# mpizenberg/visual-odometry-rs

Hardware: AMD Instinct MI355X
Metric: frame-pairs/sec (640x480, 6 pyramid levels) (higher is better)
Workload: dtype f32

## Files before the change

include/vors_hip.h:

```cpp
#ifndef VORS_HIP_H
#define VORS_HIP_H

#include <stddef.h>
#include <stdint.h>

#ifdef __cplusplus
extern "C" {
#endif

typedef enum vors_status {
    VORS_OK = 0,
    VORS_ERR_INVALID_ARGUMENT = -1,
    VORS_ERR_NO_DEVICE = -2,
    VORS_ERR_HIP = -3,
    VORS_ERR_PYRAMID_TOO_SHORT = -4,
    VORS_ERR_UNSUPPORTED = -5
} vors_status;

enum { VORS_ROW_MAJOR = 0, VORS_COL_MAJOR = 1 };

enum { VORS_CANDIDATES_COARSE_TO_FINE = 0, VORS_CANDIDATES_DENSE = 1, VORS_CANDIDATES_DSO = 2 };

enum { VORS_ARITH_REFERENCE = 0, VORS_ARITH_EXACT = 1, VORS_ARITH_FUSED = 2 };

// ... 181 lines not shown
                                 int32_t* d_out_status, vors_pair_stats* d_out_stats , void* hip_stream, int64_t* ticket);
vors_status vors_pipeline_wait(vors_pipeline* p, int64_t ticket, void* hip_stream, int host_sync);
vors_status vors_pipeline_drain(vors_pipeline* p, void* hip_stream, int host_sync);
void vors_pipeline_destroy(vors_pipeline* p);

vors_status vors_batch_get_keyframe_image(vors_batch* b, int pair, int level, uint8_t* out, int* rows, int* cols);
vors_status vors_batch_get_current_image(vors_batch* b, int pair, int level, uint8_t* out, int* rows, int* cols);
vors_status vors_batch_get_points(vors_batch* b, int pair, int level, int capacity, int32_t* xy, float* idepth, float* jac,
                                  uint8_t* tmpl, int* n);

typedef struct vors_multi vors_multi;
vors_status vors_multi_create(const vors_config* cfg, int n_devices, const int* device_ids, int max_pairs_per_device, int rows, int cols,
                              vors_multi** out);
int vors_multi_device_count(const vors_multi* m);
int vors_multi_rccl_version(const vors_multi* m);
vors_status vors_multi_shard(const vors_multi* m, int n_pairs_total, int k, int* first, int* count);
vors_status vors_multi_track_pairs(vors_multi* m, int n_pairs_total, const uint8_t* const* d_kf_gray, const uint16_t* const* d_kf_depth,
                                   const uint8_t* const* d_cur_gray, float* out_poses7, int32_t* out_status);
vors_status vors_multi_track_pairs_host(vors_multi* m, int n_pairs_total, const uint8_t* kf_gray, const uint16_t* kf_depth,
                                        const uint8_t* cur_gray, float* out_poses7, int32_t* out_status);
void vors_multi_destroy(vors_multi* m);

vors_status vors_batch_eval_level(vors_batch* b, int pair, int level, const float model7[7], int arithmetic, float sums29[29]);

enum { VORS_EVAL_FULL = 0, VORS_EVAL_ENERGY = 1 };

vors_status vors_batch_eval_pairs(vors_batch* b, int n_pairs, int level, int models_per_pair, const void* d_models, size_t model_stride_bytes,
                                  int arithmetic, int what, float* d_sums29, void* hip_stream);

vors_status vors_batch_pose_information(vors_batch* b, int n_pairs, int level, const void* d_models, size_t model_stride_bytes,
                                        float* d_info36, float* d_cov36, float* d_sigma2, int32_t* d_flags, void* hip_stream);

vors_status vors_pose_information_from_sums(const float sums29[29], float info36[36], float cov36[36], float* sigma2, int32_t* flag);

#define VORS_RESIDUAL_BINS 256
vors_status vors_batch_residual_maps(vors_batch* b, int n_pairs, int level, const void* d_models, size_t model_stride_bytes,
                                     float* d_residuals, float* d_warp_uv, uint32_t* d_hist, float* d_scale, void* hip_stream);

vors_status vors_residual_scale_from_hist(const uint32_t hist[VORS_RESIDUAL_BINS], float* median_abs, float* sigma_mad, uint32_t* n_inside);

vors_status vors_batch_reproject_depth(vors_batch* b, int n_pairs, int level, const void* d_models, size_t model_stride_bytes,
                                       const uint16_t* d_cur_depth , float tol_m,
                                       float* d_pred_z, uint16_t* d_pred_depth, float* d_depth_residual, uint32_t* d_counts,
                                       void* hip_stream);

vors_status vors_batch_point_cloud(vors_batch* b, int n_pairs, int level,
// ... 176 lines not shown
```

visual-odometry-rs_amd/csrc/batch.cpp:

```cpp
#include <algorithm>
#include <cstdlib>
#include <cstring>
#include <memory>

#include "host_common.h"

using namespace vors;

#ifndef VORS_FUSED_EXACT_POINTS_DEFAULT
#define VORS_FUSED_EXACT_POINTS_DEFAULT 2500
#endif
static vors_status build_geom(const vors_config* cfg, int rows, int cols, Geom* g) {
    if (!cfg) return fail(VORS_ERR_INVALID_ARGUMENT, "cfg is NULL");
    if (cfg->nb_levels < 1 || cfg->nb_levels > VORS_MAX_LEVELS)
        return fail(VORS_ERR_INVALID_ARGUMENT, "nb_levels must be in [1, " + std::to_string(VORS_MAX_LEVELS) + "]");
    if (rows < 2 || cols < 2 || rows > 65535 || cols > 65535) return fail(VORS_ERR_INVALID_ARGUMENT, "rows/cols must be in [2, 65535]");
    if ((long long)rows * cols > (1ll << 28))
        return fail(VORS_ERR_INVALID_ARGUMENT, "rows * cols must not exceed 2^28 pixels");
    if (cfg->candidates_mode != VORS_CANDIDATES_COARSE_TO_FINE && cfg->candidates_mode != VORS_CANDIDATES_DENSE &&
        cfg->candidates_mode != VORS_CANDIDATES_DSO)
        return fail(VORS_ERR_INVALID_ARGUMENT, "unknown candidates_mode");
    if (cfg->candidates_diff_threshold < 0 || cfg->candidates_diff_threshold > 65535)
        return fail(VORS_ERR_INVALID_ARGUMENT, "candidates_diff_threshold must fit u16");
    std::memset(g, 0, sizeof(*g));
// ... 93 lines not shown
    p.ws.mask_stride = g.S0 + g.S0 / 4 + g.S0 / 16 + 64;
    p.ws.list_cap = (g.S0 / 16 + g.S0 / 64 + g.S0 / 256 + 1024 + 3) & ~3;
    int off = 0;
    for (int l = 0; l < g.L; ++l) {
        p.pp.off[l] = off;
        if (l >= 1) off += (g.lv[l].rows * g.lv[l].cols + 3) & ~3;
    }
    p.pp.stride = off > 0 ? off : 4;
    int coff = 0;
    for (int l = 0; l < g.L; ++l) {
        p.pp.chunk_off[l] = coff;
        coff += (g.lv[l].rows * g.lv[l].cols + VORS_CHUNK_PX - 1) / VORS_CHUNK_PX;
    }
    p.pp.chunk_off[g.L] = p.pp.chunks_total = coff;
    return p;
}

struct SplitPlan {
    bool present;
    int slots;
    int chunks;
    int n_split, rounds;
    bool side_lane;
};
static SplitPlan plan_split(const Geom& g, int max_pairs) {
    SplitPlan p{};
    p.present = g.mode == VORS_CANDIDATES_DENSE && !(getenv("VORS_LM_SPLIT") && atoi(getenv("VORS_LM_SPLIT")) == 0);
    if (!p.present) return p;
    int chunks = max_pairs >= 1024 ? 64 : (max_pairs >= 512 ? 128 : 256);
    chunks = std::max(4, std::min(chunks, g.S0 / 2400));
    if (const char* ev = getenv("VORS_LM_CHUNKS")) chunks = std::max(4, atoi(ev));
    p.slots = chunks;
    int n_split = 0;
    for (int l = 0; l < g.L; ++l)
        if ((long long)g.lv[l].rows * g.lv[l].cols >= 65536) n_split = l + 1;
    p.n_split = getenv("VORS_LM_SPLIT_LEVELS") ? atoi(getenv("VORS_LM_SPLIT_LEVELS")) : std::max(1, n_split);
    p.n_split = std::max(1, std::min(p.n_split, g.L));
    if (g.arith == VORS_ARITH_FUSED)
        while (p.n_split > 0 && g.lv[p.n_split - 1].rows * g.lv[p.n_split - 1].cols <= g.fused_exact_points) p.n_split -= 1;
    const int ns = p.n_split;
    p.rounds = getenv("VORS_LM_SPLIT_ROUNDS") ? atoi(getenv("VORS_LM_SPLIT_ROUNDS")) : (max_pairs >= 512 ? (ns <= 1 ? 12 : 26) : 4 * ns + 8);
    p.chunks = p.n_split == 0 ? 0 : chunks;
    const int side_from = (getenv("VORS_LM_SIDE") && atoi(getenv("VORS_LM_SIDE")) == 1) ? 512 : 2048;
    p.side_lane = p.chunks > 0 && p.n_split == 2 && max_pairs >= side_from && !(getenv("VORS_LM_SIDE") && atoi(getenv("VORS_LM_SIDE")) == 0);
    if (p.side_lane && !getenv("VORS_LM_SPLIT_ROUNDS")) p.rounds = 10;
    return p;
}

static void allocate_workspaces(vors_batch* b) {
    const Geom& g = b->g;
    DeviceResources& own = b->own;
    const size_t np = (size_t)b->max_pairs;
    const size_t slots = np * (size_t)g.slots_total;
    own.alloc(&b->kf_upper, np * g.upper_stride);
    own.alloc(&b->cur_upper, np * g.upper_stride);
    if (g.mode == VORS_CANDIDATES_DENSE) {
        own.alloc(&b->rec.IZ, slots);
        own.alloc(&b->rec.V, slots);
        own.alloc(&b->rec.n_used, np * VORS_MAX_LEVELS);
        if (plan_ref_dense_planes(g)) {
            RefDensePlanes& t = b->rec.dense_t;
            own.alloc(&t.recs, np * ((size_t)g.S0 + g.upper_stride));
            own.alloc(&t.n_valid, np * VORS_MAX_LEVELS);
            own.alloc(&t.cur0, np * g.S0);
            own.alloc(&t.curu, np * g.upper_stride);
        }
    } else {
        own.alloc(&b->rec.S, slots);
// ... 17 lines not shown
        b->dso = plan.ws;
        b->pp = plan.pp;
        own.alloc(&b->dso.gmag, np * g.S0);
        own.alloc(&b->dso.median, np * b->dso.n_regions);
        own.alloc(&b->dso.thresh, np * b->dso.n_regions);
        own.alloc(&b->dso.max_g, np * b->dso.max_stride);
        own.alloc(&b->dso.max_pos, np * b->dso.max_stride);
        own.alloc(&b->dso.mask1, np * b->dso.mask_stride);
        own.alloc(&b->dso.picked, np * g.S0);
        own.alloc(&b->dso.state, np);
        if (own.err == hipSuccess) own.err = hipMemset(b->dso.state, 0, np * sizeof(DsoState));
        own.alloc(&b->dso.pick_list, np * (size_t)b->dso.list_cap);
        own.alloc(&b->mask0, np * g.S0);
        own.alloc(&b->pp.iz, np * b->pp.stride);
        own.alloc(&b->pp.v, np * b->pp.stride);
        own.alloc(&b->pp.counts, np * b->pp.chunks_total);
    }
    const SplitPlan sp = plan_split(g, b->max_pairs);
    if (sp.present) {
        LmSplitWs& ws = b->split;
        ws.chunks = sp.chunks;
        ws.n_split = sp.n_split;
        ws.rounds = sp.rounds;
        ws.cap = b->max_pairs;
        own.alloc(&ws.state, np);
        own.alloc(&ws.partials, np * sp.slots * 32);
        own.alloc(&ws.list[0], np);
        own.alloc(&ws.list[1], np);
        own.alloc(&ws.count, (size_t)SPLIT_COUNT_INTS);
        ws.side_round = sp.side_lane ? 1 : -1;
        if (sp.side_lane) {
            own.alloc(&ws.side_list, np);
            own.alloc(&ws.join_list, np);
            own.stream(&ws.side_stream, hipStreamNonBlocking);
            own.event(&ws.ev_fork, hipEventDisableTiming);
            own.event(&ws.ev_join, hipEventDisableTiming);
        }
    }
    if (g.mode == VORS_CANDIDATES_DENSE) {
        float2* lut = nullptr;
        own.alloc(&lut, (size_t)65536);
        b->rec.LUT = lut;
    }
}

vors_status check_stream(const vors_batch* b, hipStream_t s) {
// ... 307 lines not shown
    return VORS_OK;
}

vors_status vors_batch_eval_level(vors_batch* b, int pair, int level, const float model7[7], int arithmetic, float sums29[29]) {
    if (!b || !model7 || !sums29) return fail(VORS_ERR_INVALID_ARGUMENT, "NULL argument");
    vors_status st = check_eval(b, pair, level, arithmetic);
    if (st != VORS_OK) return st;
    DeviceGuard guard(b->device);
    DevBuf d_model, d_out;
    HIP_TRY(d_model.alloc(7 * sizeof(float)));
    HIP_TRY(d_out.alloc(32 * sizeof(float)));
    HIP_TRY(hipDeviceSynchronize());
    HIP_TRY(hipMemcpy(d_model.p, model7, 7 * sizeof(float), hipMemcpyHostToDevice));
    const EvalCall call{batch_scene(b, true), pair, level, d_model.as<float>(), d_out.as<float>()};
    if (arithmetic == VORS_ARITH_REFERENCE)
        launch_lm_eval_level_reference(b->g, call, nullptr);
    else if (arithmetic == VORS_ARITH_FUSED) launch_lm_eval_level_fused(b->g, call, nullptr);
    else launch_lm_eval_level_exact(b->g, call, nullptr);
    HIP_TRY(hipDeviceSynchronize());
    HIP_TRY(hipMemcpy(sums29, d_out.p, 29 * sizeof(float), hipMemcpyDeviceToHost));
    return VORS_OK;
}

static vors_status ensure_eval_pairs_ws(vors_batch* b) {
    EvalPairsWs& ws = b->eval_pairs;
    if (ws.items > 0) return VORS_OK;
    const int items = std::min(std::max(b->max_pairs, 256), 32768);
    int chunks = 1;
    for (int l = 0; l < b->g.L; ++l) chunks = std::max(chunks, eval_pairs_chunks(b->g, l));
    if (!ws.partials) b->own.alloc(&ws.partials, (size_t)items * chunks * 32);
    if (!ws.fctx) b->own.alloc(&ws.fctx, (size_t)items);
    if (!ws.sums29) b->own.alloc(&ws.sums29, (size_t)b->max_pairs * 29);
    if (b->own.err != hipSuccess) return own_alloc_failed(b, "evaluation workspace");
    ws.items = items;
    ws.chunks = chunks;
    return VORS_OK;
}

static vors_status batch_eval_pairs(vors_batch* b, int n_pairs, int level, int models_per_pair, const void* d_models, size_t model_stride_bytes,
                                    int arithmetic, int what, float* d_sums29, hipStream_t s) {
    vors_status st = ensure_eval_pairs_ws(b);
    if (st != VORS_OK) return st;
    EvalPairsCall call{batch_scene(b, true)};
    call.n_items = n_pairs * models_per_pair;
    call.models_per_pair = models_per_pair;
    call.lvl = level;
// ... 252 lines not shown
```

visual-odometry-rs_amd/csrc/engine.h:

```cpp
#pragma once
#include <hip/hip_runtime.h>
#include <stdint.h>

#include <type_traits>

#include "../../include/vors_hip.h"
#include "lie.h"

namespace vors {

struct LevelGeom {
    int rows, cols;
    int img_off;
    int n_slots;
    int slot_off;
    Intr k;
    FastDiv fu, fv;
    double inv_fu_d, inv_fv_d;
    float inv_fu, inv_fv, s_fuv;
};

struct Geom {
    int L;
    int mode;
// ... 71 lines not shown
};
struct DsoWs {
    uint8_t* gmag;
    uint16_t* median;
    uint16_t* thresh;
    uint8_t* max_g;
    uint32_t* max_pos;
    uint8_t* mask1;
    uint8_t* picked;
    DsoState* state;
    uint32_t* pick_list;
    int n_regions, max_stride, mask_stride, list_cap;
};
struct LmSplitState {
    float entry[7];
    float model[7];
    float cand[7];
    float sums[32];
    float cur_energy, lm_coef;
    int nb_iter;
    int n_full;
    int lvl;
    int phase;
    int went_well;
    float fctx[21];
    int fctx_exact;
};
#define VORS_SPLIT_MAX_ROUNDS 62
struct LmSplitWs {
    LmSplitState* state;
    float* partials;
    int* list[2];
    int* count;
    int cap;
    int chunks;
    int chunks0;
    int n_split;
    int rounds;
    int side_round;
    int* side_list;
    int* join_list;
    hipStream_t side_stream;
    hipEvent_t ev_fork, ev_join;
};
#define SPLIT_SIDE_COUNT (2 * (VORS_SPLIT_MAX_ROUNDS + 2))
#define SPLIT_JOIN_COUNT (2 * (VORS_SPLIT_MAX_ROUNDS + 2) + 1)
#define SPLIT_COUNT_INTS (2 * (VORS_SPLIT_MAX_ROUNDS + 2) + 2)

struct PixelPlanes {
    float* iz;
    float* v;
    int off[VORS_MAX_LEVELS];
    int stride;
    int* counts;
    int chunk_off[VORS_MAX_LEVELS + 1];
    int chunks_total;
};
constexpr int VORS_CHUNK_PX = 4096;

struct Pyramid {
    const uint8_t* level0;
// ... 472 lines not shown
```

visual-odometry-rs_amd/csrc/lm_kernels.hip:

```cpp
#include <hip/hip_runtime.h>

#include <algorithm>
#include <type_traits>

#include "lm_sources.h"

#ifndef VORS_FUSED
#define VORS_FUSED 0
#endif

namespace vors {

constexpr bool kFused = VORS_FUSED != 0;

#ifndef VORS_ABL_EXACT_STEP
#define VORS_ABL_EXACT_STEP 0
#endif
#ifndef VORS_ABL_IEEE_IDEPTH
#define VORS_ABL_IEEE_IDEPTH 0
#endif
#ifndef VORS_ABL_WIDE_IDENTITY
#define VORS_ABL_WIDE_IDENTITY 0
#endif
#ifndef VORS_ABL_IEEE_RCP
// ... 676 lines not shown
#pragma unroll
    for (int k = 0; k < 8; ++k) c[k] += __int_as_float(__builtin_amdgcn_mov_dpp(__float_as_int(c[k]), 0x104, 0xf, 0xf, true));
#pragma unroll
    for (int k = 0; k < 8; ++k) c[k] += __int_as_float(__builtin_amdgcn_mov_dpp(__float_as_int(c[k]), 0x108, 0xf, 0xf, true));
    if ((threadIdx.x & 15) < 4) {
        float4* p = reinterpret_cast<float4*>(s.part + (threadIdx.x >> 4) * 32 + (threadIdx.x & 3) * 8);
        p[0] = make_float4(c[0], c[1], c[2], c[3]);
        p[1] = make_float4(c[4], c[5], c[6], c[7]);
    }
    __syncthreads();
    if (threadIdx.x < NACC) {
        const int slot = (threadIdx.x & 3) * 8 + (threadIdx.x >> 2);
        float t = 0.f;
#pragma unroll 8
        for (int w = 0; w < BLOCK / 16; ++w) t += s.part[w * 32 + slot];
        s.sums[dst][threadIdx.x] = t;
    }
    __syncthreads();
}

template <int BLOCK>
__device__ __forceinline__ void block_sum2(float& a, float& b, LmShared& s);

__device__ __forceinline__ bool lm_step_fast(const float* h, const float* g, const Iso& model, float lm_coef, Iso* out) {
    float a[6][6], inv[6];
#pragma unroll
    for (int r = 0; r < 6; ++r)
#pragma unroll
        for (int c = 0; c <= r; ++c) a[r][c] = h[r * 6 + c];
    const float scale = 1.0f + lm_coef;
#pragma unroll
    for (int r = 0; r < 6; ++r) a[r][r] *= scale;
    bool ok = true;
#pragma unroll
    for (int j = 0; j < 6; ++j) {
#pragma unroll
        for (int k = 0; k < j; ++k) {
#pragma unroll
            for (int i = j; i < 6; ++i) a[i][j] = fmaf(-a[j][k], a[i][k], a[i][j]);
        }
        const float diag = a[j][j];
        ok = ok && (diag > 0.0f);
        inv[j] = __builtin_amdgcn_rsqf(diag);
        a[j][j] = diag * inv[j];
#pragma unroll
        for (int i = j + 1; i < 6; ++i) a[i][j] *= inv[j];
    }
    if (!ok) return false;
    float b[6];
#pragma unroll
    for (int i = 0; i < 6; ++i) b[i] = g[i];
#pragma unroll
    for (int i = 0; i < 6; ++i) {
        b[i] *= inv[i];
#pragma unroll
        for (int k = i + 1; k < 6; ++k) b[k] = fmaf(-b[i], a[k][i], b[k]);
    }
#pragma unroll
    for (int i = 5; i >= 0; --i) {
        float acc = b[i];
#pragma unroll
        for (int k = i + 1; k < 6; ++k) acc = fmaf(-a[k][i], b[k], acc);
        b[i] = acc * inv[i];
    }
    const float vx = b[0], vy = b[1], vz = b[2], wx = b[3], wy = b[4], wz = b[5];
    const float theta_2 = fmaf(wz, wz, fmaf(wy, wy, wx * wx));
    float real_factor, imag_factor, c1, c2;
    if (theta_2 < 1e-2f * 1e-2f) {
        real_factor = fmaf(-0.125f, theta_2, 1.0f);
        imag_factor = fmaf(-(1.0f / 48.0f), theta_2, 0.5f);
        c1 = fmaf(-(1.0f / 24.0f), theta_2, 0.5f);
        c2 = fmaf(-(1.0f / 120.0f), theta_2, 1.0f / 6.0f);
    } else {
        const float theta = sqrtf(theta_2), half_theta = 0.5f * theta, rt2 = 1.0f / theta_2;
        real_factor = cosf(half_theta);
        imag_factor = sinf(half_theta) / theta;
        const float sh = sinf(half_theta);
        c1 = 2.0f * sh * sh * rt2;
        c2 = (theta - sinf(theta)) * rt2 / theta;
    }
    const float w11 = wx * wx, w12 = wx * wy, w13 = wx * wz, w22 = wy * wy, w23 = wy * wz, w33 = wz * wz;
    Iso dw;
    dw.t.x = fmaf(fmaf(c2, -w22 - w33, 1.0f), vx, fmaf(fmaf(c2, w12, -c1 * wz), vy, fmaf(c2, w13, c1 * wy) * vz));
    dw.t.y = fmaf(fmaf(c2, w12, c1 * wz), vx, fmaf(fmaf(c2, -w11 - w33, 1.0f), vy, fmaf(c2, w23, -c1 * wx) * vz));
    dw.t.z = fmaf(fmaf(c2, w13, -c1 * wy), vx, fmaf(fmaf(c2, w23, c1 * wx), vy, fmaf(c2, -w11 - w22, 1.0f) * vz));
    const Quat q{imag_factor * wx, imag_factor * wy, imag_factor * wz, real_factor};
// ... 449 lines not shown
#define VORS_SPLIT_ENERGY_WAVES 8
#endif
#ifndef VORS_FSPLIT_WAVES
#define VORS_FSPLIT_WAVES 5
#endif
#ifndef VORS_FSPLIT_ENERGY_WAVES
#define VORS_FSPLIT_ENERGY_WAVES 8
#endif
template <bool HUBER, bool ENERGY, bool FUSED>
__global__ __launch_bounds__(SPLIT_BLOCK) __attribute__((amdgpu_waves_per_eu(FUSED ? (ENERGY ? VORS_FSPLIT_ENERGY_WAVES : VORS_FSPLIT_WAVES) : (ENERGY ? VORS_SPLIT_ENERGY_WAVES : VORS_SPLIT_WAVES)))) void
lm_split_eval_kernel(Geom g, const uint8_t* __restrict__ cur0, const uint8_t* __restrict__ curu, const uint8_t* __restrict__ kf0,
                     const uint8_t* __restrict__ kfu, const uint16_t* __restrict__ kf_depth, Records rec, LmSplitWs ws, int round) {
    __shared__ LmShared s;
    const int n_active = ws.count[(ENERGY ? SPLIT_COUNT_STRIDE : 0) + round], n_items = n_active * ws.chunks0;
    const int* list = ws.list[round & 1];
    for (int item = blockIdx.x; item < n_items; item += gridDim.x) {
        const int chunk = item / n_active, a = item - chunk * n_active;
        const int pair = __builtin_amdgcn_readfirstlane(ENERGY ? list[ws.cap - 1 - a] : list[a]);
        const LmSplitState* st = ws.state + pair;
        const int lvl = __builtin_amdgcn_readfirstlane(st->lvl);
        const int chunks = split_chunks(ws, lvl);
        if (chunk >= chunks) continue;
        const int phase = __builtin_amdgcn_readfirstlane(st->phase);
        const Iso model = iso_uniform(iso_load(phase == 1 ? st->cand : st->model));
        const ImgCtx c = level_ctx(g, cur0, curu, pair, lvl);
        float acc[NACC];
        float* out = ws.partials + ((size_t)pair * ws.chunks + chunk) * 32;
        with_level_source<true, true, FUSED>(g, lvl, pair, kf0, kfu, kf_depth, rec, [&](const auto& src, int n_units) {
            const LevelCut cut = level_cut(n_units, chunk, chunks);
            eval_accumulate<SPLIT_BLOCK, HUBER, false, typename std::remove_cv<typename std::remove_reference<decltype(src)>::type>::type, ENERGY>(
                src, cut.last, c, model, acc, nullptr, cut.first, FUSED ? st : nullptr);
        });
        if (ENERGY) {
            float e = acc[0], cnt = acc[1];
            block_sum2<SPLIT_BLOCK>(e, cnt, s);
            if (threadIdx.x == 0) {
                out[0] = e;
                out[1] = cnt;
            }
        } else {
            block_reduce<SPLIT_BLOCK>(acc, s, 0);
            if (threadIdx.x < NACC) out[threadIdx.x] = s.sums[0][threadIdx.x];
        }
        __syncthreads();
    }
}
#if !VORS_FUSED
template <int STEP_WAVES>
__global__ __launch_bounds__(64 * STEP_WAVES) void lm_split_step_kernel(Geom g, LmSplitWs ws, vors_pair_stats* __restrict__ out_stats, int round, int late,
                                                                        int next_late) {
    __shared__ float red_all[STEP_WAVES][32];
    __shared__ int s_kind[STEP_WAVES], s_base[3];
    const int n_active = split_n_active(ws, round);
    const int wave = threadIdx.x >> 6, lane = threadIdx.x & 63;
    float* red = red_all[wave];
    for (int a0 = blockIdx.x * STEP_WAVES; a0 < n_active; a0 += gridDim.x * STEP_WAVES) {
        const int a = a0 + wave;
        const bool live = a < n_active;
        int append_kind = -1;
        const int pair = split_active(ws, round, live ? a : 0);
        LmSplitState* st = ws.state + pair;
        const int lvl = st->lvl;
        const int chunks = split_chunks(ws, lvl);
        const int phase = st->phase;
        const bool have_full = phase != 1 || late;
        const int n_sums = have_full ? NACC : 2;
        if (live && lane < n_sums) {
            const float* pp = ws.partials + (size_t)pair * ws.chunks * 32 + lane;
            float t = 0.f;
            int ch = 0;
            for (; ch + 8 <= chunks; ch += 8) {
                float v[8];
#pragma unroll
                for (int q = 0; q < 8; ++q) v[q] = pp[(ch + q) * 32];
#pragma unroll
                for (int q = 0; q < 8; ++q) t += v[q];
            }
            for (; ch < chunks; ++ch) t += pp[ch * 32];
            red[lane] = t;
        }
        __syncthreads();
        if (live && lane == 0) {
            const float energy = red[0] / red[1];
            Iso cur_model = iso_load(st->model);
            float lm_coef = st->lm_coef, cur_energy = st->cur_energy;
            int nb_iter = st->nb_iter;
            int n_full = st->n_full;
            bool take = false, done = false, need_gh = false;
            if (phase == 0) {
                take = true;
                cur_energy = energy;
                lm_coef = 0.1f;
                nb_iter = 0;
                n_full = 1;
            } else if (phase == 4) {
                take = true;
            } else {
                const LmVerdict v = lm_verdict(energy, cur_energy, nb_iter, lm_coef);
                if (lm_accepted(v)) {
                    n_full += 1;
                    cur_energy = energy;
                    cur_model = iso_load(st->cand);
                }
                if (lm_stops(v)) done = true;
                else if (lm_accepted(v) && have_full) take = true;
                else if (lm_accepted(v)) need_gh = true;
            }
            bool again = false;
            if (done) {
                if (out_stats) store_level_stats(out_stats, pair, lvl, true, nb_iter, n_full, cur_energy);
                iso_store(cur_model, st->model);
                if (lvl > 0) {
                    iso_store(cur_model, st->entry);
                    st->lvl = lvl - 1;
                    st->phase = 0;
                    nb_iter = 0;
                    n_full = 0;
                    again = true;
                } else {
                    st->phase = 2;
                }
            } else if (need_gh) {
                iso_store(cur_model, st->model);
                st->cur_energy = cur_energy;
                st->lm_coef = lm_coef;
                st->phase = 4;
                again = true;
            } else {
                if (take) {
                    for (int q = 0; q < NACC; ++q) st->sums[q] = red[q];
                    iso_store(cur_model, st->model);
                    st->cur_energy = cur_energy;
                }
                st->lm_coef = lm_coef;
                nb_iter += 1;
                const float* sm = take ? red : st->sums;
                float h[36], gr[6];
                for (int q = 0; q < 6; ++q) gr[q] = sm[2 + q];
                int k = 8;
                for (int q = 0; q < 6; ++q)
                    for (int r = q; r < 6; ++r) {
                        h[q * 6 + r] = sm[k];
                        h[r * 6 + q] = sm[k];
                        ++k;
                    }
                Iso cand;
                if ((g.arith == VORS_ARITH_FUSED && !VORS_ABL_EXACT_STEP) ? lm_step_fast(h, gr, cur_model, lm_coef, &cand) : lm_step(h, gr, cur_model, lm_coef, &cand)) {
                    iso_store(cand, st->cand);
                    st->phase = 1;
                    again = true;
                } else {
                    for (int q = 0; q < 7; ++q) st->model[q] = st->entry[q];
                    st->went_well = 0;
                    st->phase = 2;
                    if (out_stats) zero_level_stats_below(out_stats, pair, lvl + 1);
                }
            }
            st->nb_iter = nb_iter;
            st->n_full = n_full;
            if (again && g.arith == VORS_ARITH_FUSED) store_fused_ctx(g, st->lvl, iso_load(st->phase == 1 ? st->cand : st->model), st);
            if (again) append_kind = (round == ws.side_round && st->lvl > 0) ? 2 : ((st->phase == 1 && !next_late) ? 1 : 0);
        }
        if (lane == 0) s_kind[wave] = append_kind;
        __syncthreads();
        if (threadIdx.x == 0) {
            int n_full = 0, n_energy = 0, n_side = 0;
            for (int w = 0; w < STEP_WAVES; ++w) {
                n_full += s_kind[w] == 0 ? 1 : 0;
                n_energy += s_kind[w] == 1 ? 1 : 0;
                n_side += s_kind[w] == 2 ? 1 : 0;
            }
            s_base[0] = n_full ? atomicAdd(&ws.count[round + 1], n_full) : 0;
            s_base[1] = n_energy ? atomicAdd(&ws.count[SPLIT_COUNT_STRIDE + round + 1], n_energy) : 0;
            s_base[2] = n_side ? atomicAdd(&ws.count[SPLIT_SIDE_COUNT], n_side) : 0;
        }
        __syncthreads();
        if (lane == 0 && append_kind >= 0) {
            int rank = 0;
            for (int w = 0; w < wave; ++w) rank += s_kind[w] == append_kind ? 1 : 0;
            if (append_kind == 2) ws.side_list[s_base[2] + rank] = pair;
            else if (append_kind == 1) ws.list[(round + 1) & 1][ws.cap - 1 - (s_base[1] + rank)] = pair;
            else ws.list[(round + 1) & 1][s_base[0] + rank] = pair;
        }
        __syncthreads();
    }
}

__global__ __launch_bounds__(256) void lm_split_merge_kernel(LmSplitWs ws, int round) {
    const int n = ws.count[SPLIT_JOIN_COUNT];
    for (int i = threadIdx.x; i < n; i += 256) ws.list[round & 1][atomicAdd(&ws.count[round], 1)] = ws.join_list[i];
}
void launch_lm_split_merge(LmSplitWs ws, int round, hipStream_t s) { hipLaunchKernelGGL(lm_split_merge_kernel, dim3(1), dim3(256), 0, s, ws, round); }
void launch_lm_split_step(const Geom& g, LmSplitWs ws, vors_pair_stats* out_stats, int round, int late, int next_late, int grid, hipStream_t s) {
    if (grid >= 1024 && !late)
        hipLaunchKernelGGL(lm_split_step_kernel<8>, dim3((grid + 7) / 8), dim3(512), 0, s, g, ws, out_stats, round, late, next_late);
    else
        hipLaunchKernelGGL(lm_split_step_kernel<1>, dim3(grid), dim3(64), 0, s, g, ws, out_stats, round, late, next_late);
}
#else
void launch_lm_split_merge(LmSplitWs ws, int round, hipStream_t s);
void launch_lm_split_step(const Geom& g, LmSplitWs ws, vors_pair_stats* out_stats, int round, int late, int next_late, int grid, hipStream_t s);
#endif

static void launch_lm_track_mode(const Geom& g, const TrackCall& call, int n_groups, int block, LmTrackMode mode, const LmSplitWs& split, hipStream_t s) {
    with_bool(g.mode == VORS_CANDIDATES_DENSE, [&](auto dense) {
        with_bool(g.huber_delta > 0.f, [&](auto huber) {
            with_largest_reached<1024, 512, 256, 128, 64>(block, [&](auto b) {
                constexpr int BLOCK = decltype(b)::value;
                launch_track(lm_track_kernel<BLOCK, decltype(huber)::value, decltype(dense)::value, kFused>, dim3(n_groups), dim3(BLOCK), 0, s, g, call,
                             (int)mode, split);
            });
        });
    });
}

template <bool HUBER, bool DENSE, bool FUSED>
__global__ __launch_bounds__(256) void lm_eval_level_kernel(Geom g, const uint8_t* __restrict__ cur0, const uint8_t* __restrict__ curu,
                                                             const uint8_t* __restrict__ kf0, const uint8_t* __restrict__ kfu,
                                                             const uint16_t* __restrict__ kf_depth, Records rec, int pair, int lvl,
                                                             const float* __restrict__ model7, float* __restrict__ out29) {
    __shared__ LmShared s;
    const Iso model = iso_uniform(iso_load(model7));
    const ImgCtx c = level_ctx(g, cur0, curu, pair, lvl);
    float acc[NACC];
// ... 101 lines not shown
                                      dim3(chunks, n), dim3(EVALP_BLOCK), s, g, call, item0);
                });
            });
        });
        if (chunks > 1) launch_lm_eval_pairs_sum(a, n, chunks, s);
    }
}

#if VORS_FUSED
#define VORS_LAUNCH_LM_TRACK launch_lm_track_fused
#else
#define VORS_LAUNCH_LM_TRACK launch_lm_track_exact
#endif
void VORS_LAUNCH_LM_TRACK(const Geom& g_in, const TrackCall& call, int block, LmSplitWs split, hipStream_t s) {
    const Geom g = launch_geom(g_in, call);
    const int n_pairs = call.n_pairs;
    if (g.mode != VORS_CANDIDATES_DENSE || split.chunks <= 0) {
        launch_lm_track_mode(g, call, n_pairs, block, LM_WHOLE_TRACK, split, s);
        return;
    }
    split.n_split = std::max(1, std::min(split.n_split, g.L));
    split.rounds = std::max(1, std::min(split.rounds, VORS_SPLIT_MAX_ROUNDS));
    (void)hipMemsetAsync(split.count, 0, SPLIT_COUNT_INTS * sizeof(int), s);
    const int join_round = split.side_round >= 0 ? std::min(split.side_round + 3, split.rounds) : -1;
    launch_lm_track_mode(g, call, n_pairs, block, LM_COARSE_LEVELS, split, s);
    const int base_chunks = std::max(1, split.chunks / 4);
    for (int r = 0; r < split.rounds; ++r) {
        static const int late_env = getenv("VORS_LM_LATE_FROM") ? atoi(getenv("VORS_LM_LATE_FROM")) : -1;
        const int late_from = late_env >= 0 ? late_env : 2 * split.n_split + 2;
        const int late = r >= late_from, next_late = r + 1 >= late_from;
        if (r == join_round) {
            (void)hipStreamWaitEvent(s, split.ev_join, 0);
            launch_lm_split_merge(split, r, s);
        }
        static const int late_chunks_env = getenv("VORS_LM_LATE_CHUNKS") ? atoi(getenv("VORS_LM_LATE_CHUNKS")) : 0;
        split.chunks0 = late ? (late_chunks_env > 0 ? std::min(late_chunks_env, split.chunks) : split.chunks) : base_chunks;
        const int full = n_pairs * split.chunks0;
        const int shrink = r < 2 * split.n_split ? 1 : (late ? 16 : 2);
        const int grid = std::max(std::min(full, 256), full / shrink);
        const int minor = std::max(std::min(full, 256), grid / 8);
        const int grid_full = late ? grid : ((r & 1) ? minor : grid), grid_energy = (r & 1) ? grid : minor;
        with_bool(g.huber_delta > 0.f, [&](auto huber) {
            constexpr bool HUBER = decltype(huber)::value;
            launch_on_scene(lm_split_eval_kernel<HUBER, false, kFused>, dim3(grid_full), dim3(SPLIT_BLOCK), 0, s, g, call, split, r);
            if (!late && r > 0) launch_on_scene(lm_split_eval_kernel<HUBER, true, kFused>, dim3(grid_energy), dim3(SPLIT_BLOCK), 0, s, g, call, split, r);
        });
        launch_lm_split_step(g, split, call.out_stats, r, late, next_late, std::max(1, n_pairs / shrink), s);
        if (r == split.side_round) {
            (void)hipEventRecord(split.ev_fork, s);
            (void)hipStreamWaitEvent(split.side_stream, split.ev_fork, 0);
            launch_lm_track_mode(g, call, n_pairs, 1024, LM_SIDE_LANE, split, split.side_stream);
            (void)hipEventRecord(split.ev_join, split.side_stream);
        }
    }
    if (join_round == split.rounds) {
        (void)hipStreamWaitEvent(s, split.ev_join, 0);
        launch_lm_split_merge(split, split.rounds, s);
    }
    launch_lm_track_mode(g, call, n_pairs, 1024, LM_STRAGGLERS, split, s);
    launch_lm_track_mode(g, call, n_pairs, block, LM_EPILOGUE, split, s);
}

#if !VORS_FUSED
void launch_lm_track(const Geom& g, const TrackCall& call, int block, LmSplitWs split, hipStream_t s) {
    if (g.arith == VORS_ARITH_FUSED) launch_lm_track_fused(g, call, block, split, s);
    else launch_lm_track_exact(g, call, block, split, s);
}

#define OP_BLOCK 256
__global__ void records_from_obs_kernel(Intr k, int rows, int cols, const uint8_t* __restrict__ tmpl, int n,
// ... 96 lines not shown
```

visual-odometry-rs_amd/vors_amd/__init__.py:

```python
import ctypes as C
import os
import sys

import numpy as np

_HERE = os.path.dirname(os.path.abspath(__file__))
LIB_PATH = os.environ.get("VORS_HIP_LIB") or os.path.join(_HERE, "libvors_hip.so")
MAX_LEVELS = 8
RESIDUAL_BINS = 256
RENDER_COUNTS = 4
NORMAL_COUNTS = 3
ICP_ITERATIONS, ICP_CONVERGED, ICP_TOO_FEW, ICP_SINGULAR = 0, 1, 2, 3

ROW_MAJOR, COL_MAJOR = 0, 1
CANDIDATES_COARSE_TO_FINE, CANDIDATES_DENSE, CANDIDATES_DSO = 0, 1, 2
TRACK_OK, TRACK_OPTIMIZER_FAILED_POSE_KEPT = 0, 1
ARITH_REFERENCE, ARITH_EXACT, ARITH_FUSED = 0, 1, 2


class VorsError(RuntimeError):
    pass


class vors_config(C.Structure):
# ... 41 lines not shown
    _fields_ = [
        ("cu", C.c_float), ("cv", C.c_float), ("fu", C.c_float), ("fv", C.c_float), ("skew", C.c_float),
        ("rows", C.c_int32), ("cols", C.c_int32),
        ("template_", C.POINTER(C.c_uint8)),
        ("image", C.POINTER(C.c_uint8)),
        ("n", C.c_int32),
        ("coordinates", C.POINTER(C.c_int32)),
        ("_z_candidates", C.POINTER(C.c_float)),
        ("jacobians", C.POINTER(C.c_float)),
        ("huber_delta", C.c_float),
        ("arithmetic", C.c_int32),
    ]


EXPORTED_SYMBOLS = [
    "vors_last_error", "vors_device_count", "vors_device_info", "vors_abi_version", "vors_selfcheck_isqrt",
    "vors_tracker_create", "vors_tracker_track", "vors_tracker_track_checked", "vors_tracker_current_frame", "vors_tracker_last_stats",
    "vors_tracker_keyframe", "vors_tracker_enable_depth_filter", "vors_tracker_enable_map", "vors_tracker_read_map", "vors_tracker_enable_map_voxels",
    "vors_tracker_read_map_voxels", "vors_tracker_render_map", "vors_tracker_destroy",
    "vors_track_pairs",
    "vors_batch_create", "vors_batch_create_on", "vors_batch_device", "vors_batch_track_pairs", "vors_batch_prepare_keyframes", "vors_batch_track_current",
    "vors_batch_workspace_bytes", "vors_batch_enable_kernel_timing", "vors_batch_kernel_times", "vors_batch_last_kernel_ms",
    "vors_batch_destroy",
    "vors_batch_get_keyframe_image", "vors_batch_get_current_image", "vors_batch_get_points", "vors_batch_eval_level",
    "vors_batch_eval_pairs", "vors_batch_pose_information", "vors_pose_information_from_sums",
    "vors_batch_residual_maps", "vors_residual_scale_from_hist",
    "vors_batch_reproject_depth", "vors_to_depth", "vors_from_depth",
    "vors_batch_point_cloud", "vors_camera_back_project", "vors_camera_project",
    "vors_batch_fuse_depth", "vors_fuse_depth_pixels",
    "vors_render_points", "vors_render_points_host", "vors_trackers_render_map",
    "vors_depth_normals", "vors_points_normals", "vors_depth_normals_host", "vors_trackers_enable_map_normals", "vors_trackers_map_normals",
    "vors_icp_workspace_bytes", "vors_icp_points", "vors_icp_points_host", "vors_trackers_icp_map",
    "vors_icp_points_robust", "vors_icp_points_robust_host", "vors_trackers_icp_map_robust",
    "vors_icp_points_joint", "vors_icp_points_joint_host", "vors_trackers_icp_map_joint",
    "vors_tracker_enable_map_normals", "vors_tracker_read_map_normals",
    "vors_trackers_enable_map_icp", "vors_trackers_map_icp", "vors_tracker_enable_map_icp", "vors_tracker_read_map_icp",
    "vors_map_icp_window_host", "vors_map_icp_verdict_host",
    "vors_icp_condition_from_sums", "vors_icp_condition", "vors_trackers_enable_map_icp_joint", "vors_trackers_map_icp_joint",
    "vors_tracker_enable_map_icp_joint", "vors_tracker_read_map_icp_joint", "vors_map_icp_verdict_joint_host",
    "vors_trackers_enable_map_icp_means", "vors_trackers_map_icp_means", "vors_tracker_enable_map_icp_means", "vors_tracker_read_map_icp_means",
    "vors_lm_eval", "vors_lm_step", "vors_lm_solve",
    "vors_ref_sincos", "vors_se3_exp", "vors_se3_log", "vors_so3_exp", "vors_so3_log", "vors_iso_mul", "vors_iso_inverse",
    "vors_synth_render_pairs",
    "vors_multi_create", "vors_multi_device_count", "vors_multi_shard", "vors_multi_track_pairs", "vors_multi_track_pairs_host",
    "vors_multi_destroy", "vors_multi_rccl_version",
    "vors_trackers_create", "vors_trackers_create_on", "vors_trackers_count", "vors_trackers_init", "vors_trackers_track", "vors_trackers_state",
    "vors_trackers_current_frames", "vors_trackers_last_stats", "vors_trackers_enable_kernel_timing", "vors_trackers_kernel_times", "vors_trackers_destroy",
# ... 119 lines not shown
        _lib.vors_tracker_read_map_icp_means.argtypes = [vp, vp]
        _lib.vors_voxel_keys.argtypes = [f, vp, i, vp]
        _lib.vors_voxel_keys.restype = None
        _lib.vors_synth_render_frames.argtypes = [i, vp, vp, vp, i, i, vp, i, vp, vp, vp]
        _lib.vors_batch_track_pairs.argtypes = [vp, i, vp, vp, vp, vp, vp, vp, vp, vp]
        _lib.vors_pipeline_create.argtypes = [i, C.POINTER(vors_config), i, i, i, i, C.POINTER(vp)]
        _lib.vors_pipeline_submit.argtypes = [vp, i, vp, vp, vp, vp, vp, vp, vp, vp, C.POINTER(C.c_int64)]
        _lib.vors_pipeline_wait.argtypes = [vp, C.c_int64, vp, i]
        _lib.vors_pipeline_drain.argtypes = [vp, vp, i]
        _lib.vors_pipeline_destroy.argtypes = [vp]
        _lib.vors_pipeline_destroy.restype = None
        _lib.vors_batch_prepare_keyframes.argtypes = [vp, i, vp, vp, vp]
        _lib.vors_batch_track_current.argtypes = [vp, i, vp, vp, vp, vp, vp, vp]
        _lib.vors_batch_workspace_bytes.argtypes = [vp, C.POINTER(C.c_uint64)]
        _lib.vors_batch_enable_kernel_timing.argtypes = [vp, i]
        _lib.vors_batch_kernel_times.argtypes = [vp, i, vp, i, C.POINTER(i)]
        _lib.vors_batch_last_kernel_ms.argtypes = [vp, C.POINTER(f), C.POINTER(f), C.POINTER(f)]
        _lib.vors_batch_destroy.argtypes = [vp]
        _lib.vors_batch_destroy.restype = None
        _lib.vors_batch_get_keyframe_image.argtypes = [vp, i, i, vp, C.POINTER(i), C.POINTER(i)]
        _lib.vors_batch_get_current_image.argtypes = [vp, i, i, vp, C.POINTER(i), C.POINTER(i)]
        _lib.vors_batch_get_points.argtypes = [vp, i, i, i, vp, vp, vp, vp, C.POINTER(i)]
        _lib.vors_batch_eval_level.argtypes = [vp, i, i, vp, i, vp]
        _lib.vors_batch_eval_pairs.argtypes = [vp, i, i, i, vp, C.c_size_t, i, i, vp, vp]
        _lib.vors_batch_pose_information.argtypes = [vp, i, i, vp, C.c_size_t, vp, vp, vp, vp, vp]
        _lib.vors_pose_information_from_sums.argtypes = [vp, vp, vp, C.POINTER(f), C.POINTER(C.c_int32)]
        _lib.vors_batch_residual_maps.argtypes = [vp, i, i, vp, C.c_size_t, vp, vp, vp, vp, vp]
        _lib.vors_residual_scale_from_hist.argtypes = [vp, C.POINTER(f), C.POINTER(f), C.POINTER(C.c_uint32)]
        _lib.vors_batch_reproject_depth.argtypes = [vp, i, i, vp, C.c_size_t, vp, f, vp, vp, vp, vp, vp]
        for name in ("vors_to_depth", "vors_from_depth"):
            getattr(_lib, name).argtypes = [f, vp, i, vp]
            getattr(_lib, name).restype = None
        _lib.vors_batch_point_cloud.argtypes = [vp, i, i, vp, C.c_size_t, vp, i, vp, vp, vp, vp, vp]
        _lib.vors_camera_back_project.argtypes = [vp, vp, vp, vp, i, vp]
        _lib.vors_camera_back_project.restype = None
        _lib.vors_camera_project.argtypes = [vp, vp, vp, i, vp]
        _lib.vors_camera_project.restype = None
        _lib.vors_batch_fuse_depth.argtypes = [vp, i, vp, C.c_size_t, vp, f, vp, i, i, vp, vp, vp, vp, vp]
        _lib.vors_fuse_depth_pixels.argtypes = [f, f, i, i, C.c_size_t, vp, vp, vp, C.c_size_t, vp, vp, vp]
        _lib.vors_lm_eval.argtypes = [C.POINTER(vors_obs), vp, C.POINTER(f), C.POINTER(C.c_int32), vp, vp, vp]
        _lib.vors_ref_sincos.argtypes = [vp, i, vp, vp]
        _lib.vors_ref_sincos.restype = None
        _lib.vors_lm_step.argtypes = [vp, vp, vp, f, vp, C.POINTER(i)]
        _lib.vors_lm_solve.argtypes = [C.POINTER(vors_obs), vp, vp, C.POINTER(C.c_int32), C.POINTER(f), C.POINTER(f), C.POINTER(i)]
        _lib.vors_synth_render_pairs.argtypes = [C.c_uint64, i, i, i, vp, d, i, vp, vp, vp, vp, vp, vp]
        for name in ("vors_se3_exp", "vors_se3_log", "vors_so3_exp", "vors_so3_log", "vors_iso_inverse"):
# ... 537 lines not shown
                raise VorsError(f"expected contiguous [n <= {self.max_pairs}, {self.rows}, {self.cols}] images, got {tuple(t.shape)}")

    def prepare_keyframes(self, kf_gray, kf_depth):
        n = kf_gray.shape[0]
        self._check_images(kf_gray, kf_depth)
        self._kf_refs = (kf_gray, kf_depth)
        _check(lib().vors_batch_prepare_keyframes(self._h, n, self._dp(kf_gray), self._dp(kf_depth), self._stream()))

    def track_current(self, cur_gray, out_poses7, out_status, out_stats=None, prev_poses7=None):
        n = cur_gray.shape[0]
        self._check_images(cur_gray)
        self._cur_ref = cur_gray
        _check(lib().vors_batch_track_current(self._h, n, self._dp(cur_gray), self._dp(prev_poses7), self._dp(out_poses7),
                                              self._dp(out_status), self._dp(out_stats), self._stream()))

    def track_pairs(self, kf_gray, kf_depth, cur_gray, out_poses7, out_status, out_stats=None, prev_poses7=None):
        n = kf_gray.shape[0]
        self._check_images(kf_gray, kf_depth, cur_gray)
        self._kf_refs, self._cur_ref = (kf_gray, kf_depth), cur_gray
        _check(lib().vors_batch_track_pairs(self._h, n, self._dp(kf_gray), self._dp(kf_depth), self._dp(cur_gray),
                                            self._dp(prev_poses7), self._dp(out_poses7), self._dp(out_status),
                                            self._dp(out_stats), self._stream()))

    def eval_level(self, pair, level, model7, arithmetic):
        m = np.ascontiguousarray(model7, np.float32)
        out = np.zeros(29, np.float32)
        _check(lib().vors_batch_eval_level(self._h, pair, level, _ptr(m), int(arithmetic), _ptr(out)))
        H = np.zeros((6, 6), np.float32)
        H[np.triu_indices(6)] = out[8:29]
        H = H + np.triu(H, 1).T
        return float(out[0]), int(out[1]), out[2:8].copy(), H

    @staticmethod
    def _models_arg(models):
        import torch
        if not models.is_contiguous():
            raise VorsError("models must be a contiguous tensor")
        if models.dtype == torch.uint8:
            if models.numel() % PAIR_STATS_DTYPE.itemsize != 0:
                raise VorsError("a uint8 `models` tensor must be the out_stats buffer of a track")
            return models, models.numel() // PAIR_STATS_DTYPE.itemsize, 1, PAIR_STATS_DTYPE.itemsize
        if models.dtype != torch.float32 or models.shape[-1] != 7 or models.dim() not in (2, 3):
            raise VorsError(f"expected float32 models [n, 7] or [n, K, 7], got {models.dtype} {tuple(models.shape)}")
        return models, models.shape[0], (models.shape[1] if models.dim() == 3 else 1), 0

    @staticmethod
# ... 1196 lines not shown
```

Before: 349,900.

## Speculatively evaluate full gradient/Hessian for LM candidates with large predicted decrease

When the LM step's model-predicted energy decrease (2·g·δ − δᵀHδ, normalised by point count) exceeds a threshold at the finest level, the candidate is evaluated with full Jacobian sums instead of energy-only. If it is accepted, the next step can reuse the held sums and skip a separate full-eval round. This trades extra full-accumulation work on rejected predictions for fewer sequential rounds. It also enlarges the odd-round full-eval grid and adds a prediction log with a debug API.

```diff
diff --git a/include/vors_hip.h b/include/vors_hip.h
--- a/include/vors_hip.h
+++ b/include/vors_hip.h
@@ -227,6 +227,13 @@
 void vors_multi_destroy(vors_multi* m);
 
 vors_status vors_batch_eval_level(vors_batch* b, int pair, int level, const float model7[7], int arithmetic, float sums29[29]);
+
+#define VORS_PREDICT_FULL 1
+#define VORS_PREDICT_FULL_GO_ON 2
+#define VORS_PREDICT_FULL_STOP 4
+#define VORS_PREDICT_FULL_REJECTED 8
+#define VORS_PREDICT_MISSED 16
+vors_status vors_batch_lm_predict_log(vors_batch* b, int n_pairs, int32_t* log);
 
 enum { VORS_EVAL_FULL = 0, VORS_EVAL_ENERGY = 1 };
 
diff --git a/visual-odometry-rs_amd/csrc/batch.cpp b/visual-odometry-rs_amd/csrc/batch.cpp
--- a/visual-odometry-rs_amd/csrc/batch.cpp
+++ b/visual-odometry-rs_amd/csrc/batch.cpp
@@ -139,6 +139,8 @@
     int chunks;
     int n_split, rounds;
     bool side_lane;
+    bool predict;
+    float predict_tau;
 };
 static SplitPlan plan_split(const Geom& g, int max_pairs) {
     SplitPlan p{};
@@ -161,6 +163,8 @@
     const int side_from = (getenv("VORS_LM_SIDE") && atoi(getenv("VORS_LM_SIDE")) == 1) ? 512 : 2048;
     p.side_lane = p.chunks > 0 && p.n_split == 2 && max_pairs >= side_from && !(getenv("VORS_LM_SIDE") && atoi(getenv("VORS_LM_SIDE")) == 0);
     if (p.side_lane && !getenv("VORS_LM_SPLIT_ROUNDS")) p.rounds = 10;
+    p.predict = p.chunks > 0 && g.arith == VORS_ARITH_FUSED && !(getenv("VORS_LM_PREDICT") && atoi(getenv("VORS_LM_PREDICT")) == 0);
+    p.predict_tau = getenv("VORS_LM_PREDICT_TAU") ? (float)atof(getenv("VORS_LM_PREDICT_TAU")) : VORS_LM_PREDICT_TAU;
     return p;
 }
 
@@ -224,6 +228,9 @@
         ws.chunks = sp.chunks;
         ws.n_split = sp.n_split;
         ws.rounds = sp.rounds;
+        ws.predict = sp.predict ? 1 : 0;
+        ws.predict_tau = sp.predict_tau;
+        if (sp.predict) own.alloc(&ws.pred_log, np);
         ws.cap = b->max_pairs;
         own.alloc(&ws.state, np);
         own.alloc(&ws.partials, np * sp.slots * 32);
@@ -577,6 +584,19 @@
     return VORS_OK;
 }
 
+vors_status vors_batch_lm_predict_log(vors_batch* b, int n_pairs, int32_t* log) {
+    if (!b || !log) return fail(VORS_ERR_INVALID_ARGUMENT, "NULL argument");
+    if (n_pairs < 0 || n_pairs > b->max_pairs) return fail(VORS_ERR_INVALID_ARGUMENT, "n_pairs out of range");
+    DeviceGuard guard(b->device);
+    HIP_TRY(hipDeviceSynchronize());
+    if (!b->split.pred_log) {
+        for (int i = 0; i < n_pairs; ++i) log[i] = 0;
+        return VORS_OK;
+    }
+    HIP_TRY(hipMemcpy(log, b->split.pred_log, (size_t)n_pairs * sizeof(int32_t), hipMemcpyDeviceToHost));
+    return VORS_OK;
+}
+
 static vors_status ensure_eval_pairs_ws(vors_batch* b) {
     EvalPairsWs& ws = b->eval_pairs;
     if (ws.items > 0) return VORS_OK;
diff --git a/visual-odometry-rs_amd/csrc/engine.h b/visual-odometry-rs_amd/csrc/engine.h
--- a/visual-odometry-rs_amd/csrc/engine.h
+++ b/visual-odometry-rs_amd/csrc/engine.h
@@ -117,11 +117,13 @@
     int n_full;
     int lvl;
     int phase;
+    int pred;
     int went_well;
     float fctx[21];
     int fctx_exact;
 };
 #define VORS_SPLIT_MAX_ROUNDS 62
+#define VORS_LM_PREDICT_TAU 1.0f
 struct LmSplitWs {
     LmSplitState* state;
     float* partials;
@@ -132,6 +134,9 @@
     int chunks0;
     int n_split;
     int rounds;
+    int predict;
+    float predict_tau;
+    int* pred_log;
     int side_round;
     int* side_list;
     int* join_list;
diff --git a/visual-odometry-rs_amd/csrc/lm_kernels.hip b/visual-odometry-rs_amd/csrc/lm_kernels.hip
--- a/visual-odometry-rs_amd/csrc/lm_kernels.hip
+++ b/visual-odometry-rs_amd/csrc/lm_kernels.hip
@@ -722,7 +722,7 @@
 template <int BLOCK>
 __device__ __forceinline__ void block_sum2(float& a, float& b, LmShared& s);
 
-__device__ __forceinline__ bool lm_step_fast(const float* h, const float* g, const Iso& model, float lm_coef, Iso* out) {
+__device__ __forceinline__ bool lm_step_fast(const float* h, const float* g, const Iso& model, float lm_coef, Iso* out, float* delta_out = nullptr) {
     float a[6][6], inv[6];
 #pragma unroll
     for (int r = 0; r < 6; ++r)
@@ -762,6 +762,10 @@
 #pragma unroll
         for (int k = i + 1; k < 6; ++k) acc = fmaf(-a[k][i], b[k], acc);
         b[i] = acc * inv[i];
+    }
+    if (delta_out) {
+#pragma unroll
+        for (int i = 0; i < 6; ++i) delta_out[i] = b[i];
     }
     const float vx = b[0], vy = b[1], vz = b[2], wx = b[3], wy = b[4], wz = b[5];
     const float theta_2 = fmaf(wz, wz, fmaf(wy, wy, wx * wx));
@@ -1257,6 +1261,9 @@
         const int chunks = split_chunks(ws, lvl);
         if (chunk >= chunks) continue;
         const int phase = __builtin_amdgcn_readfirstlane(st->phase);
+        const int pred = ENERGY ? 0 : __builtin_amdgcn_readfirstlane(st->pred);
+        if (!ENERGY && phase == 4 && pred == 2) continue;
+        const bool energy_order = !ENERGY && phase == 1 && pred == 1;
         const Iso model = iso_uniform(iso_load(phase == 1 ? st->cand : st->model));
         const ImgCtx c = level_ctx(g, cur0, curu, pair, lvl);
         float acc[NACC];
@@ -1274,16 +1281,32 @@
                 out[1] = cnt;
             }
         } else {
+            float e = acc[0], cnt = acc[1];
+            if (energy_order) block_sum2<SPLIT_BLOCK>(e, cnt, s);
             block_reduce<SPLIT_BLOCK>(acc, s, 0);
             if (threadIdx.x < NACC) out[threadIdx.x] = s.sums[0][threadIdx.x];
+            if (energy_order && threadIdx.x == 0) {
+                out[0] = e;
+                out[1] = cnt;
+            }
         }
         __syncthreads();
     }
 }
 #if !VORS_FUSED
+__device__ __forceinline__ float lm_promised_decrease(const float* h36, const float* g6, const float* delta, float n) {
+    float gd = 0.f, dhd = 0.f;
+    for (int q = 0; q < 6; ++q) {
+        float hd = 0.f;
+        for (int r = 0; r < 6; ++r) hd = fmaf(h36[q * 6 + r], delta[r], hd);
+        gd = fmaf(g6[q], delta[q], gd);
+        dhd = fmaf(delta[q], hd, dhd);
+    }
+    return (2.0f * gd - dhd) / n;
+}
 template <int STEP_WAVES>
 __global__ __launch_bounds__(64 * STEP_WAVES) void lm_split_step_kernel(Geom g, LmSplitWs ws, vors_pair_stats* __restrict__ out_stats, int round, int late,
-                                                                        int next_late) {
+                                                                        int next_late, int predict) {
     __shared__ float red_all[STEP_WAVES][32];
     __shared__ int s_kind[STEP_WAVES], s_base[3];
     const int n_active = split_n_active(ws, round);
@@ -1298,8 +1321,10 @@
         const int lvl = st->lvl;
         const int chunks = split_chunks(ws, lvl);
         const int phase = st->phase;
-        const bool have_full = phase != 1 || late;
-        const int n_sums = have_full ? NACC : 2;
+        const int pred = (phase == 1 || phase == 4) ? st->pred : 0;
+        const bool held = phase == 4 && pred == 2;
+        const bool have_full = phase != 1 || late || pred == 1;
+        const int n_sums = held ? 0 : (have_full ? NACC : 2);
         if (live && lane < n_sums) {
             const float* pp = ws.partials + (size_t)pair * ws.chunks * 32 + lane;
             float t = 0.f;
@@ -1316,12 +1341,13 @@
         }
         __syncthreads();
         if (live && lane == 0) {
-            const float energy = red[0] / red[1];
+            const float energy = held ? 0.f : red[0] / red[1];
+            int log_bits = 0;
             Iso cur_model = iso_load(st->model);
             float lm_coef = st->lm_coef, cur_energy = st->cur_energy;
             int nb_iter = st->nb_iter;
             int n_full = st->n_full;
-            bool take = false, done = false, need_gh = false;
+            bool take = false, done = false, need_gh = false, hold = false;
             if (phase == 0) {
                 take = true;
                 cur_energy = energy;
@@ -1329,7 +1355,7 @@
                 nb_iter = 0;
                 n_full = 1;
             } else if (phase == 4) {
-                take = true;
+                take = !held;
             } else {
                 const LmVerdict v = lm_verdict(energy, cur_energy, nb_iter, lm_coef);
                 if (lm_accepted(v)) {
@@ -1338,10 +1364,13 @@
                     cur_model = iso_load(st->cand);
                 }
                 if (lm_stops(v)) done = true;
+                else if (lm_accepted(v) && pred == 1) hold = true;
                 else if (lm_accepted(v) && have_full) take = true;
                 else if (lm_accepted(v)) need_gh = true;
-            }
-            bool again = false;
+                if (pred == 1) log_bits |= hold ? VORS_PREDICT_FULL_GO_ON : (lm_accepted(v) ? VORS_PREDICT_FULL_STOP : VORS_PREDICT_FULL_REJECTED);
+                if (pred == 3 && need_gh) log_bits |= VORS_PREDICT_MISSED;
+            }
+            bool again = false, go_full = false;
             if (done) {
                 if (out_stats) store_level_stats(out_stats, pair, lvl, true, nb_iter, n_full, cur_energy);
                 iso_store(cur_model, st->model);
@@ -1355,11 +1384,14 @@
                 } else {
                     st->phase = 2;
                 }
-            } else if (need_gh) {
+            } else if (need_gh || hold) {
+                if (hold)
+                    for (int q = 0; q < NACC; ++q) st->sums[q] = red[q];
                 iso_store(cur_model, st->model);
                 st->cur_energy = cur_energy;
                 st->lm_coef = lm_coef;
                 st->phase = 4;
+                st->pred = hold ? 2 : 0;
                 again = true;
             } else {
                 if (take) {
@@ -1380,9 +1412,14 @@
                         ++k;
                     }
                 Iso cand;
-                if ((g.arith == VORS_ARITH_FUSED && !VORS_ABL_EXACT_STEP) ? lm_step_fast(h, gr, cur_model, lm_coef, &cand) : lm_step(h, gr, cur_model, lm_coef, &cand)) {
+                float delta[6] = {0.f, 0.f, 0.f, 0.f, 0.f, 0.f};
+                if ((g.arith == VORS_ARITH_FUSED && !VORS_ABL_EXACT_STEP) ? lm_step_fast(h, gr, cur_model, lm_coef, &cand, delta) : lm_step(h, gr, cur_model, lm_coef, &cand)) {
                     iso_store(cand, st->cand);
                     st->phase = 1;
+                    const bool may = predict && lvl == 0 && !lm_too_many_iterations(nb_iter);
+                    go_full = may && lm_promised_decrease(h, gr, delta, sm[1]) > ws.predict_tau;
+                    st->pred = go_full ? 1 : (may ? 3 : 0);
+                    if (go_full) log_bits |= VORS_PREDICT_FULL;
                     again = true;
                 } else {
                     for (int q = 0; q < 7; ++q) st->model[q] = st->entry[q];
@@ -1393,8 +1430,9 @@
             }
             st->nb_iter = nb_iter;
             st->n_full = n_full;
+            if (ws.pred_log && log_bits) ws.pred_log[pair] |= log_bits;
             if (again && g.arith == VORS_ARITH_FUSED) store_fused_ctx(g, st->lvl, iso_load(st->phase == 1 ? st->cand : st->model), st);
-            if (again) append_kind = (round == ws.side_round && st->lvl > 0) ? 2 : ((st->phase == 1 && !next_late) ? 1 : 0);
+            if (again) append_kind = (round == ws.side_round && st->lvl > 0) ? 2 : ((st->phase == 1 && !next_late && !go_full) ? 1 : 0);
         }
         if (lane == 0) s_kind[wave] = append_kind;
         __syncthreads();
@@ -1426,15 +1464,17 @@
     for (int i = threadIdx.x; i < n; i += 256) ws.list[round & 1][atomicAdd(&ws.count[round], 1)] = ws.join_list[i];
 }
 void launch_lm_split_merge(LmSplitWs ws, int round, hipStream_t s) { hipLaunchKernelGGL(lm_split_merge_kernel, dim3(1), dim3(256), 0, s, ws, round); }
-void launch_lm_split_step(const Geom& g, LmSplitWs ws, vors_pair_stats* out_stats, int round, int late, int next_late, int grid, hipStream_t s) {
+void launch_lm_split_step(const Geom& g, LmSplitWs ws, vors_pair_stats* out_stats, int round, int late, int next_late, int predict, int grid,
+                          hipStream_t s) {
     if (grid >= 1024 && !late)
-        hipLaunchKernelGGL(lm_split_step_kernel<8>, dim3((grid + 7) / 8), dim3(512), 0, s, g, ws, out_stats, round, late, next_late);
+        hipLaunchKernelGGL(lm_split_step_kernel<8>, dim3((grid + 7) / 8), dim3(512), 0, s, g, ws, out_stats, round, late, next_late, predict);
     else
-        hipLaunchKernelGGL(lm_split_step_kernel<1>, dim3(grid), dim3(64), 0, s, g, ws, out_stats, round, late, next_late);
+        hipLaunchKernelGGL(lm_split_step_kernel<1>, dim3(grid), dim3(64), 0, s, g, ws, out_stats, round, late, next_late, predict);
 }
 #else
 void launch_lm_split_merge(LmSplitWs ws, int round, hipStream_t s);
-void launch_lm_split_step(const Geom& g, LmSplitWs ws, vors_pair_stats* out_stats, int round, int late, int next_late, int grid, hipStream_t s);
+void launch_lm_split_step(const Geom& g, LmSplitWs ws, vors_pair_stats* out_stats, int round, int late, int next_late, int predict, int grid,
+                          hipStream_t s);
 #endif
 
 static void launch_lm_track_mode(const Geom& g, const TrackCall& call, int n_groups, int block, LmTrackMode mode, const LmSplitWs& split, hipStream_t s) {
@@ -1582,6 +1622,7 @@
     split.n_split = std::max(1, std::min(split.n_split, g.L));
     split.rounds = std::max(1, std::min(split.rounds, VORS_SPLIT_MAX_ROUNDS));
     (void)hipMemsetAsync(split.count, 0, SPLIT_COUNT_INTS * sizeof(int), s);
+    if (split.pred_log) (void)hipMemsetAsync(split.pred_log, 0, (size_t)n_pairs * sizeof(int), s);
     const int join_round = split.side_round >= 0 ? std::min(split.side_round + 3, split.rounds) : -1;
     launch_lm_track_mode(g, call, n_pairs, block, LM_COARSE_LEVELS, split, s);
     const int base_chunks = std::max(1, split.chunks / 4);
@@ -1599,13 +1640,16 @@
         const int shrink = r < 2 * split.n_split ? 1 : (late ? 16 : 2);
         const int grid = std::max(std::min(full, 256), full / shrink);
         const int minor = std::max(std::min(full, 256), grid / 8);
-        const int grid_full = late ? grid : ((r & 1) ? minor : grid), grid_energy = (r & 1) ? grid : minor;
+        static const int pred_div_env = getenv("VORS_LM_PREDICT_GRID_DIV") ? std::max(1, atoi(getenv("VORS_LM_PREDICT_GRID_DIV"))) : 0;
+        const int minor_full = (split.predict && r >= 2 && r + 1 < std::min(late_from, split.rounds)) ? std::max(minor, grid / (pred_div_env ? pred_div_env : 8)) : minor;
+        const int grid_full = late ? grid : ((r & 1) ? minor_full : grid), grid_energy = (r & 1) ? grid : minor;
         with_bool(g.huber_delta > 0.f, [&](auto huber) {
             constexpr bool HUBER = decltype(huber)::value;
             launch_on_scene(lm_split_eval_kernel<HUBER, false, kFused>, dim3(grid_full), dim3(SPLIT_BLOCK), 0, s, g, call, split, r);
             if (!late && r > 0) launch_on_scene(lm_split_eval_kernel<HUBER, true, kFused>, dim3(grid_energy), dim3(SPLIT_BLOCK), 0, s, g, call, split, r);
         });
-        launch_lm_split_step(g, split, call.out_stats, r, late, next_late, std::max(1, n_pairs / shrink), s);
+        const int predict = split.predict && r + 2 < std::min(late_from, split.rounds);
+        launch_lm_split_step(g, split, call.out_stats, r, late, next_late, predict, std::max(1, n_pairs / shrink), s);
         if (r == split.side_round) {
             (void)hipEventRecord(split.ev_fork, s);
             (void)hipStreamWaitEvent(split.side_stream, split.ev_fork, 0);
diff --git a/visual-odometry-rs_amd/vors_amd/__init__.py b/visual-odometry-rs_amd/vors_amd/__init__.py
--- a/visual-odometry-rs_amd/vors_amd/__init__.py
+++ b/visual-odometry-rs_amd/vors_amd/__init__.py
@@ -87,7 +87,7 @@
     "vors_batch_create", "vors_batch_create_on", "vors_batch_device", "vors_batch_track_pairs", "vors_batch_prepare_keyframes", "vors_batch_track_current",
     "vors_batch_workspace_bytes", "vors_batch_enable_kernel_timing", "vors_batch_kernel_times", "vors_batch_last_kernel_ms",
     "vors_batch_destroy",
-    "vors_batch_get_keyframe_image", "vors_batch_get_current_image", "vors_batch_get_points", "vors_batch_eval_level",
+    "vors_batch_get_keyframe_image", "vors_batch_get_current_image", "vors_batch_get_points", "vors_batch_eval_level", "vors_batch_lm_predict_log",
     "vors_batch_eval_pairs", "vors_batch_pose_information", "vors_pose_information_from_sums",
     "vors_batch_residual_maps", "vors_residual_scale_from_hist",
     "vors_batch_reproject_depth", "vors_to_depth", "vors_from_depth",
@@ -253,6 +253,7 @@
         _lib.vors_batch_get_current_image.argtypes = [vp, i, i, vp, C.POINTER(i), C.POINTER(i)]
         _lib.vors_batch_get_points.argtypes = [vp, i, i, i, vp, vp, vp, vp, C.POINTER(i)]
         _lib.vors_batch_eval_level.argtypes = [vp, i, i, vp, i, vp]
+        _lib.vors_batch_lm_predict_log.argtypes = [vp, i, vp]
         _lib.vors_batch_eval_pairs.argtypes = [vp, i, i, i, vp, C.c_size_t, i, i, vp, vp]
         _lib.vors_batch_pose_information.argtypes = [vp, i, i, vp, C.c_size_t, vp, vp, vp, vp, vp]
         _lib.vors_pose_information_from_sums.argtypes = [vp, vp, vp, C.POINTER(f), C.POINTER(C.c_int32)]
@@ -836,6 +837,11 @@
                                             self._dp(prev_poses7), self._dp(out_poses7), self._dp(out_status),
                                             self._dp(out_stats), self._stream()))
 
+    def lm_predict_log(self, n_pairs):
+        out = np.zeros(n_pairs, np.int32)
+        _check(lib().vors_batch_lm_predict_log(self._h, n_pairs, _ptr(out)))
+        return out
+
     def eval_level(self, pair, level, model7, arithmetic):
         m = np.ascontiguousarray(model7, np.float32)
         out = np.zeros(29, np.float32)
```

Result: faster. 359,800 (median of 6 runs) (+2.8%).
